# dojo-sim/Dojo.jl

Hardware: NVIDIA H100
Metric: env-steps/sec (forward step!) (higher is better)
Workload: dtype f64

## Files before the change

### dojo.jl_b200/csrc/dojo_b200.cu

```cuda
#include <cuda_runtime.h>

#include <algorithm>
#include <climits>
#include <cstdio>
#include <cstdlib>
#include <cstring>
#include <string>
#include <vector>

#include "../../include/dojo_b200.h"
#include "dojo_step_kernel.cuh"
#include "dojo_kin.cuh"
#include "dojo_kinjac.cuh"
#include "dojo_envs.cuh"
#include "dojo_storage.cuh"

using namespace dj;

extern "C" __attribute__((visibility("hidden"))) const void* dojo_cm_step_kernel(int grad);
static const void* step_kernel_fn(bool any_contact, bool grad, bool plan_smem, bool small = false) {
  if (any_contact) return dojo_cm_step_kernel(grad ? 1 : 0);
  if (plan_smem && !getenv("DOJO_B200_GENERIC_PLAN")) {
    if (!grad && small) return (const void*)dojo_step_kernel<false, true, false, true>;
    return grad ? (const void*)dojo_step_kernel<true, true> : (const void*)dojo_step_kernel<false, true>;
// ... 390 lines not shown
    auto slot_entry = [&](const JointDev& J, int slot) { return (J.flags & JF_FULL) ? (slot | (1 << 30)) : slot; };
    ilist.push_back(slot_entry(joints[parent_joint[b]], joints[parent_joint[b]].slot_c));
    for (int j = 0; j < Ne; ++j) if (joints[j].parent == b) ilist.push_back(slot_entry(joints[j], joints[j].slot_p));
    bodies[b].g_cnt = (int)ilist.size() - bodies[b].g_off;
  }

  for (int b = 0; b < Nb; ++b) {
    bodies[b].pjoint = parent_joint[b];
    bodies[b].cj_off = (int)ilist.size();
    for (int j = 0; j < Ne; ++j) if (joints[j].parent == b) ilist.push_back(j);
    bodies[b].cj_cnt = (int)ilist.size() - bodies[b].cj_off;
    bodies[b].ct_off = (int)ilist.size();
    for (int c = 0; c < Ni; ++c) if (contacts[c].body == b) ilist.push_back(c);
    bodies[b].ct_cnt = (int)ilist.size() - bodies[b].ct_off;
  }

  std::vector<WarpRole> roles(nw);
  {
    for (auto& r : roles) std::memset(&r, 0, sizeof(r));
    auto add = [&](int w, int type, int first, int count) {
      if (count <= 0) return;
      WarpRole& r = roles[w];
      r.type[r.npass] = type; r.first[r.npass] = first; r.count[r.npass] = count; r.npass++;
    };
    if (nw == 1) { add(0, ROLE_BODY, 0, Nb); add(0, ROLE_CONTACT, 0, Ni); add(0, ROLE_JOINT, 0, Ne); }
    else if (nw == 2) { add(0, ROLE_BODY, 0, Nb); add(0, ROLE_CONTACT, 0, Ni); add(1, ROLE_JOINT, 0, Ne); }
    else if (nw == 4) {
      const int hb = (Nb + 1) / 2, hc = (Ni + 1) / 2, hj = (Ne + 1) / 2;
      add(0, ROLE_BODY, 0, hb); add(0, ROLE_CONTACT, 0, hc);
      add(1, ROLE_BODY, hb, Nb - hb); add(1, ROLE_CONTACT, hc, Ni - hc);
      add(2, ROLE_JOINT, 0, hj); add(3, ROLE_JOINT, hj, Ne - hj);
    }
    else {
      int hb = (Nb + 1) / 2, hc = (Ni + 1) / 2, qj = (Ne + 3) / 4;
      add(0, ROLE_BODY, 0, hb); add(1, ROLE_BODY, hb, Nb - hb);
      add(2, ROLE_CONTACT, 0, hc); add(3, ROLE_CONTACT, hc, Ni - hc);
      for (int q = 0; q < 4; ++q) add(4 + q, ROLE_JOINT, q * qj, std::max(0, std::min(qj, Ne - q * qj)));
    }
  }

  struct HStep { ElimStep s; int height; int group; double cost; };
  std::vector<HStep> hs;
  std::vector<int> body_height(Nb, 0);
  {
    std::vector<char> done(Nb, 0);
    struct Rec {
      std::vector<JointDev>& joints; std::vector<BodyDev>& bodies; std::vector<ContactDev>& contacts;
      const std::vector<int>& pj; std::vector<char>& done; std::vector<HStep>& hs; std::vector<int>& ilist; int Ne, Ni;
      int visit(int b) {
        done[b] = 1;
        int hb = 0;
        std::vector<int> fold, gfold;
        for (int j = 0; j < Ne; ++j)
          if (joints[j].parent == b && !done[joints[j].child]) {
            int hc = visit(joints[j].child);
            hb = std::max(hb, hc + 1);
            fold.push_back(joints[j].S_off);
            gfold.push_back(joints[j].gv_off);
          }
        const BodyDev& B = bodies[b];
        const JointDev& J = joints[pj[b]];
        {
          HStep h; std::memset(&h, 0, sizeof(h));
          ElimStep& s = h.s;
          s.d_off = B.D_off; s.n = 6; s.vec_off = B.sol_off; s.r_off = B.r_off; s.nnb = 0;
          s.fold_off = (int)ilist.size(); s.fold_cnt = (int)fold.size();
          for (int f : fold) ilist.push_back(f);
          s.gfold_off = (int)ilist.size();
          for (int f : gfold) ilist.push_back(f);
          int ij = -1, ip = -1;
          if (joint_nq(J) > 0) {
            ij = s.nnb++;
            s.nb[ij].n = joint_nq(J); s.nb[ij].vec_off = J.sol_off; s.nb[ij].r_off = J.r_off; s.nb[ij].gv_off = -1; s.nb[ij].fwd_abs = -1; s.nb[ij].L_off = J.Uc_off; s.nb[ij].U_off = J.Lc_off; s.nb[ij].U_k = 6; s.nb[ij].U_row = 0;
            s.nb[ij].ld = joint_nq(J); s.nb[ij].row0 = 0;
          }
          int r0 = 0;
          if (J.parent >= 0 && J.BBpc_off >= 0) {
            ip = s.nnb++;
            const BodyDev& Pb = bodies[J.parent];
            r0 = (J.flags & JF_FULL) ? 0 : 3;
            s.nb[ip].n = 6 - r0; s.nb[ip].vec_off = Pb.sol_off + r0; s.nb[ip].r_off = Pb.r_off + r0; s.nb[ip].gv_off = J.gv_off; s.nb[ip].fwd_abs = J.S_off + 36 + r0;
            s.nb[ip].L_off = J.BBpc_off; s.nb[ip].U_off = J.BBcp_off; s.nb[ip].U_k = 6 - r0; s.nb[ip].U_row = r0;
            s.nb[ip].ld = 6; s.nb[ip].row0 = r0;
          }
          if (ij >= 0) s.tgt[ij][ij] = J.D_off;
          if (ip >= 0) s.tgt[ip][ip] = J.S_off + 7 * r0;
          if (ij >= 0 && ip >= 0) { s.tgt[ij][ip] = J.Up_off + r0; s.tgt[ip][ij] = J.Lp_off + r0 * joint_nq(J); }
          h.height = hb; h.group = -1; h.cost = 4.0 + joint_nq(J) * 0.3;
          hs.push_back(h);
        }
        int hj = hb;
        if (joint_nq(J) > 0) {
          HStep h; std::memset(&h, 0, sizeof(h));
          ElimStep& s = h.s;
          s.d_off = J.D_off; s.n = joint_nq(J); s.vec_off = J.sol_off; s.r_off = J.r_off; s.nnb = 0;
          if (J.parent >= 0) {
            const BodyDev& Pb = bodies[J.parent];
            s.nnb = 1;
            s.nb[0].n = 6; s.nb[0].vec_off = Pb.sol_off; s.nb[0].r_off = Pb.r_off; s.nb[0].gv_off = J.gv_off; s.nb[0].fwd_abs = J.S_off + 36; s.nb[0].L_off = J.Lp_off; s.nb[0].U_off = J.Up_off; s.nb[0].U_k = joint_nq(J); s.nb[0].U_row = 0;
            s.nb[0].ld = 6; s.nb[0].row0 = 0;
            s.tgt[0][0] = J.S_off;
          }
          hj = hb + 1;
          h.height = hj; h.group = -1; h.cost = 2.0 + joint_nq(J) * 0.4;
          hs.push_back(h);
        }
        return hj;
      }
    } rec{joints, bodies, contacts, parent_joint, done, hs, ilist, Ne, Ni};
    for (int j = 0; j < Ne; ++j) if (joints[j].parent < 0 && !done[joints[j].child]) rec.visit(joints[j].child);
    for (int b = 0; b < Nb; ++b) if (!done[b]) { delete h; return fail("mechanism is not a tree rooted at the origin"); }
  }
  int nphase = 0;
  for (auto& x : hs) nphase = std::max(nphase, x.height + 1);
  std::vector<ElimStep> steps;
  std::vector<int> sched((size_t)nphase * nw * 2, 0);
  for (int ph = 0; ph < nphase; ++ph) {
    std::vector<std::vector<int>> per_warp(nw);
    std::vector<double> load(nw, 0.0);
    std::vector<int> group_warp(Nb, -1);
    for (int i = 0; i < (int)hs.size(); ++i) {
      if (hs[i].height != ph) continue;
      int w;
      if (hs[i].group >= 0 && group_warp[hs[i].group] >= 0) w = group_warp[hs[i].group];
      else {
        w = 0;
        for (int k = 1; k < nw; ++k) if (load[k] < load[w]) w = k;
        if (hs[i].group >= 0) group_warp[hs[i].group] = w;
      }
      per_warp[w].push_back(i);
      load[w] += hs[i].cost;
    }
    for (int w = 0; w < nw; ++w) {
      sched[2 * (ph * nw + w)] = (int)steps.size();
      sched[2 * (ph * nw + w) + 1] = (int)per_warp[w].size();
      for (int i : per_warp[w]) steps.push_back(hs[i].s);
    }
  }
  P.nphase = nphase;
  h->nsteps = (int)steps.size();
  {
    std::vector<int> cnt((size_t)nphase * nw), wfirst(nw);
    std::vector<LduOp> ops;
    bool fits = true;
    auto u16 = [&](int v) { fits = fits && v >= 0 && v < kLduNone; return v & 0xffff; };
    auto u8 = [&](int v) { fits = fits && v >= 0 && v < 256; return v & 0xff; };
    for (int w = 0; w < nw; ++w) {
      wfirst[w] = (int)ops.size();
      for (int ph = 0; ph < nphase; ++ph) {
        const int s0 = sched[2 * (ph * nw + w)], sn = sched[2 * (ph * nw + w) + 1];
        cnt[ph * nw + w] = sn;
        for (int s = s0; s < s0 + sn; ++s) {
          const ElimStep& st = steps[s];
          int f[kLduFold] = {0, 0, 0};
          for (int k = 0; k < std::min(st.fold_cnt, kLduFold); ++k) f[k] = ilist[st.fold_off + k];
          LduOp op;
          std::memset(&op, 0, sizeof(op));
          op.w[0] = u16(st.d_off) | u16(st.vec_off) << 16;
          op.w[1] = u8(st.n) | u8(st.nnb) << 8 | u16(st.fold_cnt) << 16;
          op.w[2] = u16(st.fold_off) | u16(f[0]) << 16;
          op.w[3] = u16(f[1]) | u16(f[2]) << 16;
          for (int i = 0; i < st.nnb; ++i) {
            const ElimNb& nb = st.nb[i];
            int* q = op.w + 4 * (1 + i);
            q[0] = u16(nb.L_off) | (nb.fwd_abs >= 0 ? u16(nb.fwd_abs) : kLduNone) << 16;
            q[1] = u16(nb.vec_off) | u16(nb.U_off) << 16;
            q[2] = u8(nb.n) | u8(nb.U_row) << 8 | u8(nb.U_k) << 16 | u8(nb.ld) << 24;
            q[3] = u16(st.tgt[i][0]) | (st.nnb > 1 ? u16(st.tgt[i][1]) : 0) << 16;
          }
          ops.push_back(op);
        }
      }
    }
    if (!fits) { delete h; return fail("the block LDU program does not fit its 16-bit offsets"); }
    P.prog_cnt = (int)sched.size();
    sched.insert(sched.end(), cnt.begin(), cnt.end());
    sched.insert(sched.end(), wfirst.begin(), wfirst.end());
    sched.resize((sched.size() + 3) & ~size_t(3), 0);
    P.prog_ops = (int)sched.size();
    const int* words = reinterpret_cast<const int*>(ops.data());
    sched.insert(sched.end(), words, words + ops.size() * (sizeof(LduOp) / sizeof(int)));
  }

  cudaDeviceProp prop;
  if (cudaGetDeviceProperties(&prop, device) != cudaSuccess) { delete h; g_create_error = "cudaGetDeviceProperties failed"; return DOJO_ECUDA; }
  h->sm_count = prop.multiProcessorCount;
  if (h->arena_bytes > (size_t)prop.sharedMemPerBlockOptin) {
    delete h;
    g_create_error = "dojo_create: mechanism does not fit the per-environment shared-memory arena";
    return DOJO_ENOMEM;
  }
  auto upload = [&](const void* src, size_t bytes, void** dst) -> bool {
    if (bytes == 0) { *dst = nullptr; return true; }
    if (cudaMalloc(dst, bytes) != cudaSuccess) return false;
    return cudaMemcpy(*dst, src, bytes, cudaMemcpyHostToDevice) == cudaSuccess;
  };
  std::vector<char> blob;
  {
    const void* src[8] = {bodies.data(), joints.data(), contacts.data(), steps.data(), sched.data(), ilist.data(), roles.data(), ucol.data()};
    const size_t len[8] = {sizeof(BodyDev) * Nb, sizeof(JointDev) * Ne, sizeof(ContactDev) * Ni, sizeof(ElimStep) * steps.size(), sizeof(int) * sched.size(),
                           sizeof(int) * ilist.size(), sizeof(WarpRole) * roles.size(), sizeof(int) * ucol.size()};
    const int order[8] = {4, 3, 5, 6, 7, 0, 2, 1};
    for (int q = 0; q < 8; ++q) {
      const int k = order[q];
      h->blob_off[k] = (int)blob.size();
      blob.insert(blob.end(), (const char*)src[k], (const char*)src[k] + len[k]);
      blob.resize((blob.size() + 15) & ~size_t(15), 0);
      h->blob_end[k] = (int)blob.size();
    }
    h->blob_bytes = (int)blob.size();
  }
  bool ok = upload(blob.data(), blob.size(), (void**)&h->d_blob);
  {
    std::vector<int> order;
    std::vector<char> placed(Nb, 0), used(Ne, 0);
    for (bool progress = true; progress && (int)order.size() < Ne;) {
      progress = false;
      for (int j = 0; j < Ne; ++j)
        if (!used[j] && (joints[j].parent < 0 || placed[joints[j].parent])) { order.push_back(j); used[j] = 1; placed[joints[j].child] = 1; progress = true; }
    }
    ok = ok && (int)order.size() == Ne && upload(order.data(), sizeof(int) * Ne, (void**)&h->d_kin_order);
  }
  ok = ok && cudaMalloc((void**)&h->d_counter, sizeof(int)) == cudaSuccess;
  ok = ok && cudaMalloc((void**)&h->d_order, sizeof(int) * max_batch) == cudaSuccess && cudaMalloc((void**)&h->d_prev_iters, sizeof(int32_t) * max_batch) == cudaSuccess &&
       cudaMemset(h->d_prev_iters, 0, sizeof(int32_t) * max_batch) == cudaSuccess;
  if (const char* e = getenv("DOJO_B200_LPT")) { h->lpt = atoi(e) != 0; h->lpt_mode = atoi(e); }
  ok = ok && cudaMalloc((void**)&h->d_key, sizeof(int32_t) * max_batch) == cudaSuccess;
  ok = ok && cudaMalloc((void**)&h->d_prof, (32 + 2 * (size_t)max_batch) * sizeof(unsigned long long)) == cudaSuccess && cudaMemset(h->d_prof, 0, 32 * sizeof(unsigned long long)) == cudaSuccess &&
       cudaMemset(h->d_prof + 31, 0xff, sizeof(unsigned long long)) == cudaSuccess;
  ok = ok && cudaStreamCreateWithFlags(&h->stream, cudaStreamNonBlocking) == cudaSuccess;
  ok = ok && cudaEventCreateWithFlags(&h->ev_last, cudaEventDisableTiming) == cudaSuccess;
  auto pick_slots = [&](size_t bytes) {
    int g = (int)std::min<size_t>((size_t)prop.sharedMemPerBlockOptin / bytes, (size_t)(256 / (32 * nw)));
    g = std::max(1, std::min(g, 8));
    if (const char* e = getenv("DOJO_B200_SLOTS")) { int v = atoi(e); if (v >= 1 && v <= g) g = v; }
    return g;
  };
  h->slots = pick_slots(h->arena_bytes);
  const bool smem_plan = !getenv("DOJO_B200_GLOBAL_PLAN");
  auto plan_prefix = [&](int n, size_t bytes, int* off, int* pbytes, int* mask) {
    *off = -1; *pbytes = 0; *mask = 0;
    if (!smem_plan) return;
    const size_t room = (size_t)prop.sharedMemPerBlockOptin - 1024 - n * bytes;
    for (int k = 0; k < 8; ++k)
      if ((size_t)h->blob_end[k] <= room) { *mask |= 1 << k; *pbytes = std::max(*pbytes, h->blob_end[k]); }
    for (int k = 0; k < 8; ++k)
      if (((*mask >> k) & 1) && h->blob_end[k] > *pbytes) *mask &= ~(1 << k);
    if (*mask) *off = (int)(n * bytes / sizeof(double));
  };
  plan_prefix(h->slots, h->arena_bytes, &h->plan_smem_off, &h->plan_smem_bytes, &h->plan_smem_mask);
  h->smem_fwd = h->slots * h->arena_bytes + h->plan_smem_bytes;
  h->small_step = small_step_ok(h, h->plan_smem_mask);
  h->k_fwd = step_kernel_fn(h->any_contact, false, h->plan_smem_mask == 0xff, h->small_step);
  h->k_grad = step_kernel_fn(h->any_contact, true, false);
  ok = ok && max_shared_memory(h->k_fwd, device) == cudaSuccess;
  const bool grad_fits = h->grad_bytes <= (size_t)prop.sharedMemPerBlockOptin;
  if (grad_fits) {
    h->slots_grad = pick_slots(h->grad_bytes);
    plan_prefix(h->slots_grad, h->grad_bytes, &h->plan_smem_off_grad, &h->plan_smem_bytes_grad, &h->plan_smem_mask_grad);
    h->smem_grad = h->slots_grad * h->grad_bytes + h->plan_smem_bytes_grad;
    h->k_grad = step_kernel_fn(h->any_contact, true, h->plan_smem_mask_grad == 0xff);
    ok = ok && max_shared_memory(h->k_grad, device) == cudaSuccess;
  } else h->grad_bytes = 0;
  if (!ok) { g_create_error = std::string("dojo_create: device allocation failed: ") + cudaGetErrorString(cudaGetLastError()); dojo_destroy(h); return DOJO_ECUDA; }
  P.bodies = (const BodyDev*)(h->d_blob + h->blob_off[0]); P.joints = (const JointDev*)(h->d_blob + h->blob_off[1]);
  P.contacts = (const ContactDev*)(h->d_blob + h->blob_off[2]); P.steps = (const ElimStep*)(h->d_blob + h->blob_off[3]);
  P.sched = (const int*)(h->d_blob + h->blob_off[4]); P.ilist = (const int*)(h->d_blob + h->blob_off[5]);
  P.roles = (const WarpRole*)(h->d_blob + h->blob_off[6]); P.ucol = (const int*)(h->d_blob + h->blob_off[7]);
  int occ = 1;
  cudaOccupancyMaxActiveBlocksPerMultiprocessor(&occ, h->k_fwd, 32 * h->nw * h->slots, h->smem_fwd);
  h->envs_per_sm = std::max(1, occ);
  if (h->grad_bytes) { occ = 1; cudaOccupancyMaxActiveBlocksPerMultiprocessor(&occ, h->k_grad, 32 * h->nw * h->slots_grad, h->smem_grad); h->envs_per_sm_grad = std::max(1, occ); }
  *out = h;
  return DOJO_OK;
}

extern "C" int dojo_destroy(DojoHandle* h) {
  if (!h) return DOJO_OK;
  cudaSetDevice(h->device);
  cudaFree(h->d_key); cudaFree(h->d_order); cudaFree(h->d_prev_iters); cudaFree(h->d_prof); cudaFree(h->d_blob); cudaFree(h->d_counter); cudaFree(h->d_kin_order); cudaFree(h->d_kjws); cudaFree(h->d_kjout); cudaFree(h->d_recZ[0]); cudaFree(h->d_recZ[1]); cudaFree(h->d_recS); cudaFree(h->d_recD); cudaFree(h->d_recAny); cudaFree(h->d_envTheta); cudaFree(h->d_envNorm); cudaFree(h->d_envS); cudaFree(h->d_envSn); cudaFree(h->d_envA); cudaFree(h->d_envR); cudaFree(h->d_envS0); cudaFree(h->d_envDone); cudaFree(h->d_X); cudaFree(h->d_Xn); cudaFree(h->d_gsol); cudaFree(h->d_gstatus); cudaFree(h->d_done); cudaFree(h->d_trace);
  for (int k = 0; k < 2; ++k) { cudaFree(h->d_Fz[k]); cudaFree(h->d_Fu[k]); if (h->ev_kernel[k]) cudaEventDestroy(h->ev_kernel[k]); if (h->ev_copy[k]) cudaEventDestroy(h->ev_copy[k]); }
  if (h->copy_stream) cudaStreamDestroy(h->copy_stream);
  cudaFree(h->d_Z); cudaFree(h->d_U); cudaFree(h->d_F); cudaFree(h->d_Zn); cudaFree(h->d_sol); cudaFree(h->d_status); cudaFree(h->d_iters);
  if (h->p_in) cudaFreeHost(h->p_in);
  if (h->p_out) cudaFreeHost(h->p_out);
  if (h->stream) cudaStreamDestroy(h->stream);
  if (h->ev_last) cudaEventDestroy(h->ev_last);
  cudaFree(h->d_rollU); cudaFree(h->d_rollTraj);
  cudaFree(h->d_rsol); cudaFree(h->d_rdone); cudaFree(h->d_rstatus); cudaFree(h->d_riters); cudaFree(h->d_rZ); cudaFree(h->d_rU); cudaFree(h->d_rX);
  delete h;
  return DOJO_OK;
}

extern "C" const char* dojo_last_error(const DojoHandle* h) { return h ? h->err.c_str() : g_create_error.c_str(); }
extern "C" int dojo_num_state(const DojoHandle* h) { return h->plan.nz; }
extern "C" int dojo_num_input(const DojoHandle* h) { return h->plan.nu; }
extern "C" int dojo_num_residual(const DojoHandle* h) { return h->plan.nres; }
extern "C" int dojo_num_grad_state(const DojoHandle* h) { return 12 * h->plan.Nb; }
extern "C" int dojo_shared_bytes_per_env(const DojoHandle* h) { return (int)h->arena_bytes; }
extern "C" int64_t dojo_launch_count(const DojoHandle* h) { return h->launches; }
extern "C" int dojo_debug_config(const DojoHandle* h, int* out) {
  if (!h || !out) return DOJO_EINVAL;
  const int v[17] = {h->slots, h->slots_grad, h->plan.ch, (int)h->arena_bytes, (int)h->grad_bytes, (int)h->smem_fwd, (int)h->smem_grad,
                     h->plan_smem_mask, h->plan_smem_mask_grad, h->plan.ls_pair, h->plan.nphase, h->nsteps, h->blob_bytes, h->nw, h->envs_per_sm,
                     h->envs_per_sm_grad, h->small_step ? 1 : 0};
  for (int i = 0; i < 17; ++i) out[i] = v[i];
// ... 1224 lines not shown
```

### dojo.jl_b200/csrc/dojo_kernels.cuh

```cuda
#pragma once
#include "dojo_linalg.cuh"
#include "dojo_plan.h"

namespace dj {

#ifdef DJ_ANY_CONTACT
#define DJ_SLOT_OFF(raw) ((raw) & 0x3fffffff)
#define DJ_SLOT_FULL(raw) (((raw) >> 30) & 1)
#else
#define DJ_SLOT_OFF(raw) (raw)
#endif
#ifdef DJ_ANY_CONTACT
DJ_DEV int contact_type(const ContactDev& cd) { return cd.tn & 0xff; }
DJ_DEV int contact_nh(const ContactDev& cd) { return cd.tn >> 8; }
#endif

DJ_DEV V3 ld3(const double* p) { return V3{p[0], p[1], p[2]}; }
DJ_DEV void st3(double* p, V3 v) { p[0] = v.x; p[1] = v.y; p[2] = v.z; }
DJ_DEV void add3(double* p, V3 v) { p[0] += v.x; p[1] += v.y; p[2] += v.z; }
DJ_DEV M33 ldm33(const double* p) {
  M33 r;
#pragma unroll
  for (int i = 0; i < 3; ++i)
#pragma unroll
// ... 1009 lines not shown
      const LimitSide ls = limit_side(so[is_u], so[is_l], so[ig_u], so[ig_l]);
      const double* lim = A + jd.lim_off + kLim * i;
      const double adw = dot(ld3(lim), wp) + dot(ld3(lim + 3), wc);
      const double dgA = xr[is_u], rcI = xr[is_l], rs_u = xr[ig_u], rs_l = xr[ig_l];
      const double ds_u = rs_u - adw, ds_l = rs_l + adw;
      const double dgI = (rcI - ls.gI * (ls.up ? ds_l : ds_u)) / ls.sI;
      xr[is_u] = ds_u;
      xr[is_l] = ds_l;
      xr[ig_u] = ls.up ? dgA : dgI;
      xr[ig_l] = ls.up ? dgI : dgA;
    }
  }
}

template <bool JAC, bool SMALL = false>
DJ_DEV void evaluate(Ctx& c, double f, int res_off, double& rvio, double& bvio) {
  const Plan& P = *c.P;
  double* A = c.A;
  double* res = A + res_off;
  const WarpRole& role = c.roles[c.warp];
  double rv = 0.0, bv = 0.0;
  if (JAC) {
    for (int t = c.tid; t < P.mat_len; t += c.nthreads) A[P.mat_off + t] = 0.0;
    slot_sync(c);
  }
  for (int p = 0; p < role.npass; ++p) {
    if (JAC && role.type[p] == ROLE_JOINT && (SMALL || (P.jpair && role.count[p] <= 16))) {
      if ((c.lane >> 1) < role.count[p]) eval_joint_pair(c, role.first[p] + (c.lane >> 1), (c.lane & 1) != 0, res, rv, bv);
      continue;
    }
    const int idx = role_item(role, p, c.lane);
    if (idx < 0) continue;
    if (role.type[p] == ROLE_BODY) eval_body<JAC>(c, idx, f, res);
    else if (role.type[p] == ROLE_CONTACT) eval_contact<JAC>(c, idx, f, res, rv, bv);
    else if (!(SMALL && JAC)) eval_joint<JAC>(c, idx, f, res, rv, bv);
  }
#ifdef DJ_PROFILE
  long long _rw0 = clock64();
#endif
  slot_sync(c);
#ifdef DJ_PROFILE
  c.t_rolewait += clock64() - _rw0;
#endif
  for (int p = 0; p < role.npass; ++p) {
    const int idx = role_item(role, p, c.lane);
    if (idx < 0 || role.type[p] != ROLE_BODY) continue;
    const BodyDev& bd = c.bodies[idx];
    double* rb = res + bd.sol_off;
    double* D = A + bd.D_off;
    for (int g = 0; g < bd.g_cnt; ++g) {
      const double* s = A + DJ_SLOT_OFF(c.ilist[bd.g_off + g]);
      add3(rb, ld3(s));
      add3(rb + 3, ld3(s + 3));
      if (JAC) {
#ifdef DJ_ANY_CONTACT
        if (g < bd.g_ncontact || DJ_SLOT_FULL(c.ilist[bd.g_off + g])) {
#else
        if (g < bd.g_ncontact) {
#endif
#pragma unroll
          for (int i = 0; i < 36; ++i) D[i] -= s[6 + i];
        } else {
#pragma unroll
          for (int i = 0; i < 3; ++i)
#pragma unroll
            for (int j = 0; j < 3; ++j) D[(3 + i) * 6 + 3 + j] -= s[6 + 3 * i + j];
        }
      }
    }
#pragma unroll
    for (int i = 0; i < 6; ++i) rv = nanmax(rv, fabs(rb[i]));
  }
  block_nanmax2<SMALL>(c, rv, bv);
  rvio = rv;
  bvio = bv;
  slot_sync(c);
}

template <bool SMALL = false>
DJ_DEV void evaluate_ls(Ctx& c, double* W, double fk, bool pair, double& rvA, double& bvA, double& rvB, double& bvB) {
  const Plan& P = *c.P;
  double* A = c.A;
  const WarpRole& role = c.roles[c.warp];
  const bool pl = SMALL || P.ls_pair != 0;
  const int half = pl ? (c.lane >> 4) : 0;
  const int ln = pl ? (c.lane & 15) : c.lane;
  const bool on = (half == 0) || pair;
  const double f = half ? 0.5 * fk : fk;
  double* res = W + (half ? P.ls_res2_off : P.sav_off);
  c.sd = (int)(W - A) + (half ? P.ls_slot_delta : 0);
  double rv = 0.0, bv = 0.0;
  for (int p = 0; p < role.npass; ++p) {
    const int idx = on ? role_item(role, p, ln) : -1;
    if (idx < 0) continue;
    if (role.type[p] == ROLE_BODY) eval_body<false>(c, idx, f, res);
    else if (role.type[p] == ROLE_CONTACT) eval_contact<false>(c, idx, f, res, rv, bv);
    else eval_joint<false>(c, idx, f, res, rv, bv);
  }
  slot_sync(c);
  for (int p = 0; p < role.npass; ++p) {
    const int idx = on ? role_item(role, p, ln) : -1;
    if (idx < 0 || role.type[p] != ROLE_BODY) continue;
    const BodyDev& bd = c.bodies[idx];
    double* rb = res + bd.sol_off;
    for (int g = 0; g < bd.g_cnt; ++g) {
      const double* s = A + DJ_SLOT_OFF(c.ilist[bd.g_off + g]) + c.sd;
      add3(rb, ld3(s));
      add3(rb + 3, ld3(s + 3));
    }
#pragma unroll
    for (int i = 0; i < 6; ++i) rv = nanmax(rv, fabs(rb[i]));
  }
  c.sd = 0;
#pragma unroll
  for (int o = 8; o > 0; o >>= 1) {
    rv = nanmax(rv, __shfl_xor_sync(0xffffffffu, rv, o));
    bv = nanmax(bv, __shfl_xor_sync(0xffffffffu, bv, o));
  }
  if (!pl) {
    rv = nanmax(rv, __shfl_xor_sync(0xffffffffu, rv, 16));
    bv = nanmax(bv, __shfl_xor_sync(0xffffffffu, bv, 16));
  }
  double* red = W + P.red_off;
  if ((c.lane & 15) == 0) { red[4 * c.warp + 2 * (c.lane >> 4)] = rv; red[4 * c.warp + 2 * (c.lane >> 4) + 1] = bv; }
  slot_sync(c);
  rvA = red[0]; bvA = red[1]; rvB = red[2]; bvB = red[3];
  for (int w = 1; w < slot_warps<SMALL>(c); ++w) {
    rvA = nanmax(rvA, red[4 * w]); bvA = nanmax(bvA, red[4 * w + 1]);
    rvB = nanmax(rvB, red[4 * w + 2]); bvB = nanmax(bvB, red[4 * w + 3]);
  }
  slot_sync(c);
}

DJ_DEV const int* ldu_cnt(const Ctx& c) { return c.sched + c.P->prog_cnt; }
DJ_DEV const int4* ldu_op(const Ctx& c, int k) { return reinterpret_cast<const int4*>(c.sched + c.P->prog_ops) + 3 * k; }
DJ_DEV int ldu_fold(const Ctx& c, int4 h, int j) {
  return j == 0 ? hi16(h.z) : j == 1 ? lo16(h.w) : j == 2 ? hi16(h.w) : c.ilist[lo16(h.z) + j];
}
static_assert(kLduFold == 3, "ldu_fold names three inline fold sources");

template <bool SMALL = false>
DJ_DEV bool factorize(Ctx& c) {
  const Plan& P = *c.P;
  double* A = c.A;
  bool ok = true;
  const int half = c.lane >> 4, l = c.lane & 15;
  const unsigned mask = 0xffffu << (16 * half);
  const int nw = slot_warps<SMALL>(c);
  const int* cnt = ldu_cnt(c);
  int k = cnt[P.nphase * nw + c.warp];
#ifdef DJ_PROFILE
  c.f_last = clock64();
#endif
  for (int ph = 0; ph < P.nphase; ++ph) {
    const int sn = cnt[ph * nw + c.warp];
    for (int s = half; s < sn; s += 2) {
      const int4* q = ldu_op(c, k + s);
      const int4 h = q[0];
      const int n = byte_of(h.y, 0), nnb = byte_of(h.y, 1), fold_cnt = hi16(h.y);
      double* Dc = A + lo16(h.x);
      if (fold_cnt > 0) {
        for (int t = l; t < n * n; t += 16) {
          double acc = Dc[t];
          for (int j = 0; j < fold_cnt; ++j) acc += A[ldu_fold(c, h, j) + t];
          Dc[t] = acc;
        }
        __syncwarp(mask);
      }
      DJ_FTICK(c, f_fold)
      ok = block_inverse(Dc, n, n, l, mask) && ok;
      DJ_FTICK(c, f_inv)
      for (int i = 0; i < nnb; ++i) {
        const int4 a = q[1 + i];
        right_multiply_inplace(A + lo16(a.x), Dc, byte_of(a.z, 0), n, l, mask);
      }
      DJ_FTICK(c, f_rm)
      for (int i = 0; i < nnb; ++i)
        for (int j = 0; j < nnb; ++j) {
          const int4 ai = q[1 + i], aj = q[1 + j];
          schur_update(A + (j ? hi16(ai.w) : lo16(ai.w)), byte_of(aj.z, 3), A + lo16(ai.x) + byte_of(aj.z, 1), n, A + hi16(aj.y), byte_of(ai.z, 0),
                       byte_of(aj.z, 2), byte_of(aj.z, 0), l, mask);
        }
      DJ_FTICK(c, f_schur)
    }
    k += sn;
    slot_sync(c);
    DJ_FTICK(c, f_bar)
  }
  int* flag = (int*)(A + P.red_off);
  const bool wok = __all_sync(0xffffffffu, ok);
  if (c.lane == 0) flag[c.warp] = wok ? 1 : 0;
  slot_sync(c);
  bool all = true;
  for (int w = 0; w < slot_warps<SMALL>(c); ++w) all = all && (flag[w] != 0);
  slot_sync(c);
  return all;
}

DJ_DEV double dot6(const double* a, const double* b, int n) {
  double e = 0.0, o = 0.0;
#pragma unroll
  for (int k = 0; k < 6; k += 2) {
    if (k < n) e = fma(a[k], b[k], e);
    if (k + 1 < n) o = fma(a[k + 1], b[k + 1], o);
  }
  return e + o;
}

template <bool SMALL = false>
DJ_DEV void solve(Ctx& c, int vec_off) {
  const Plan& P = *c.P;
  double* A = c.A;
  double* x = A + vec_off;
  const int lane = c.lane;
  const int half = lane >> 4, l = lane & 15;
  const int sub = l >> 3, li = l & 7;
  const WarpRole& role = c.roles[c.warp];
#ifdef DJ_PROFILE
  c.f_last = clock64();
#endif
  for (int p = 0; p < role.npass; ++p) {
    const int idx = role_item(role, p, lane);
    if (idx < 0) continue;
    if (role.type[p] == ROLE_CONTACT) condense_contact(c, idx, x);
    else if (role.type[p] == ROLE_JOINT) condense_joint(c, idx, x);
  }
  DJ_FTICK(c, s_cond)
  slot_sync(c);
  DJ_FTICK(c, s_bar)
  for (int p = 0; p < role.npass; ++p) {
    const int idx = role_item(role, p, lane);
    if (idx < 0 || role.type[p] != ROLE_BODY) continue;
    const BodyDev& bd = c.bodies[idx];
    double* xb = x + bd.sol_off;
    for (int g = 0; g < bd.g_cnt; ++g) {
      const double* s = A + DJ_SLOT_OFF(c.ilist[bd.g_off + g]);
      add3(xb, ld3(s));
      add3(xb + 3, ld3(s + 3));
    }
  }
  DJ_FTICK(c, s_cond)
  slot_sync(c);
  DJ_FTICK(c, s_bar)
  const int nw = slot_warps<SMALL>(c);
  const int* cnt = ldu_cnt(c);
  int k = cnt[P.nphase * nw + c.warp];
  for (int ph = 0; ph < P.nphase; ++ph) {
    const int sn = cnt[ph * nw + c.warp];
    for (int it = 0; 2 * it < sn; ++it) {
      const bool act = 2 * it + half < sn;
      const int4* q = ldu_op(c, k + 2 * it + (act ? half : 0));
      const int4 h = q[0];
      const int n = byte_of(h.y, 0), fold_cnt = hi16(h.y);
      double* xc = x + hi16(h.x);
      if (act && fold_cnt > 0 && l < n) {
        double acc = xc[l];
        for (int j = 0; j < fold_cnt; ++j) {
          double* v = A + ldu_fold(c, h, j) + 36;
          acc += v[l];
          v[l] = 0.0;
        }
        xc[l] = acc;
      }
      __syncwarp();
      if (act && sub < byte_of(h.y, 1)) {
        const int4 a = q[1 + sub];
        if (li < byte_of(a.z, 0)) {
          const double* L = A + lo16(a.x) + li * n;
          const double acc = dot6(L, xc, n);
          double* tgt = hi16(a.x) != kLduNone ? A + hi16(a.x) : x + lo16(a.y);
          tgt[li] -= acc;
        }
      }
      __syncwarp();
    }
    k += sn;
    DJ_FTICK(c, s_fwd)
    slot_sync(c);
    DJ_FTICK(c, s_bar)
  }
  for (int ph = P.nphase - 1; ph >= 0; --ph) {
    const int sn = cnt[ph * nw + c.warp];
    k -= sn;
    for (int it = (sn + 1) / 2 - 1; it >= 0; --it) {
      const bool act = 2 * it + half < sn;
      const int4* q = ldu_op(c, k + 2 * it + (act ? half : 0));
      const int4 h = q[0];
      const int n = byte_of(h.y, 0), nnb = byte_of(h.y, 1);
      const double* Dc = A + lo16(h.x);
      double* xc = x + hi16(h.x);
      if (act && nnb > 0 && l < n) {
        double acc = 0.0;
        for (int j = 0; j < nnb; ++j) {
          const int4 a = q[1 + j];
          const int nn = byte_of(a.z, 0), r = l - byte_of(a.z, 1);
          if (r >= 0 && r < byte_of(a.z, 2)) {
            acc += dot6(A + hi16(a.y) + r * nn, x + lo16(a.y), nn);
          }
        }
        xc[l] -= acc;
      }
      __syncwarp();
      double acc = 0.0;
      if (act && l < n) acc = dot6(Dc + l * n, xc, n);
      __syncwarp();
      if (act && l < n) xc[l] = acc;
      __syncwarp();
    }
    DJ_FTICK(c, s_bwd)
    slot_sync(c);
    DJ_FTICK(c, s_bar)
  }
  for (int p = 0; p < role.npass; ++p) {
    const int idx = role_item(role, p, lane);
    if (idx < 0) continue;
    if (role.type[p] == ROLE_CONTACT) recover_contact(c, idx, x);
    else if (role.type[p] == ROLE_JOINT) recover_joint(c, idx, x);
  }
  DJ_FTICK(c, s_rec)
  slot_sync(c);
  DJ_FTICK(c, s_bar)
}

DJ_DEV double ort_step(double lam, double dl, double tau) { return dl < 0.0 ? fmin(1.0, -tau * lam / dl) : 1.0; }
DJ_DEV double soc_step(double l0, double l1, double l2, double d0, double d1, double d2, double tau) {
  const double eps = 1e-14;
  double ll = fmax(l0 * l0 - (l1 * l1 + l2 * l2), 1e-25) + eps;
  double ld = l0 * d0 - (l1 * d1 + l2 * d2) + eps;
  double rs = ld / ll;
  double sq = sqrt(ll);
  double fct = (ld / sq + d0) / (l0 / sq + 1.0);
  double r1 = d1 / sq - fct * l1 / ll;
  double r2 = d2 / sq - fct * l2 / ll;
  double nr = sqrt(r1 * r1 + r2 * r2);
  return (nr - rs > 0.0) ? fmin(1.0, tau / (nr - rs)) : 1.0;
}
template <bool SMALL = false>
DJ_DEV double cone_line_search(Ctx& c, double tau_ort, double tau_soc) {
  const Plan& P = *c.P;
  const double* sol = c.A + P.sol_off;
  const double* dl = c.A + P.rhs_off;
  const WarpRole& role = c.roles[c.warp];
  double a = 1.0;
  for (int p = 0; p < role.npass; ++p) {
#ifndef DJ_ANY_CONTACT
    if (role.type[p] == ROLE_CONTACT && role.count[p] <= 16) {
      const int ci = c.lane >> 1;
      if (ci < role.count[p]) {
        const ContactDev& cd = c.contacts[role.first[p] + ci];
        const int o = cd.sol_off + 4 * (c.lane & 1);
        const double* v = sol + o;
        const double* dv = dl + o;
        a = fmin(a, ort_step(v[0], dv[0], tau_ort));
        a = fmin(a, soc_step(v[1], v[2], v[3], dv[1], dv[2], dv[3], tau_soc));
      }
      continue;
    }
#endif
    const int idx = role_item(role, p, c.lane);
    if (idx < 0) continue;
    if (role.type[p] == ROLE_CONTACT) {
      const ContactDev& cd = c.contacts[idx];
      const double* s = sol + cd.sol_off;
#ifdef DJ_ANY_CONTACT
      if (contact_type(cd) != 2) {
        const int n2 = 2 * contact_nh(cd);
        for (int i = 0; i < n2; ++i) a = fmin(a, ort_step(s[i], dl[cd.sol_off + i], tau_ort));
        continue;
      }
#endif
      const double* g = s + 4;
      const double* ds = dl + cd.sol_off;
      const double* dg = ds + 4;
      a = fmin(a, ort_step(s[0], ds[0], tau_ort));
      a = fmin(a, ort_step(g[0], dg[0], tau_ort));
      a = fmin(a, soc_step(s[1], s[2], s[3], ds[1], ds[2], ds[3], tau_soc));
      a = fmin(a, soc_step(g[1], g[2], g[3], dg[1], dg[2], dg[3], tau_soc));
    } else if (role.type[p] == ROLE_JOINT) {
      const JointDev& jd = c.joints[idx];
      for (int i = 0; i < 2 * jd.nb_r; ++i) a = fmin(a, ort_step(sol[jd.sol_off + jd.ne + i], dl[jd.sol_off + jd.ne + i], tau_ort));
    }
  }
  return block_min<SMALL>(c, a);
}

template <bool SMALL = false>
DJ_DEV void centering(Ctx& c, double aaff, double& nu, double& nuaff) {
  const Plan& P = *c.P;
  const double* sol = c.A + P.sol_off;
  const double* dl = c.A + P.rhs_off;
  const WarpRole& role = c.roles[c.warp];
  double sn = 0.0, sa = 0.0, cnt = 0.0;
  for (int p = 0; p < role.npass; ++p) {
    const int idx = role_item(role, p, c.lane);
    if (idx < 0) continue;
    if (role.type[p] == ROLE_CONTACT) {
      const ContactDev& cd = c.contacts[idx];
#ifdef DJ_ANY_CONTACT
      if (contact_type(cd) != 2) {
        const int nh = contact_nh(cd);
        for (int i = 0; i < nh; ++i) {
          double s = sol[cd.sol_off + i], g = sol[cd.sol_off + nh + i];
          sn += s * g;
          sa += (s + aaff * dl[cd.sol_off + i]) * (g + aaff * dl[cd.sol_off + nh + i]);
        }
        cnt += (double)nh;
        continue;
      }
#endif
#pragma unroll
      for (int i = 0; i < 4; ++i) {
        double s = sol[cd.sol_off + i], g = sol[cd.sol_off + 4 + i];
        sn += s * g;
        sa += (s + aaff * dl[cd.sol_off + i]) * (g + aaff * dl[cd.sol_off + 4 + i]);
      }
      cnt += 2.0;
    } else if (role.type[p] == ROLE_JOINT) {
      const JointDev& jd = c.joints[idx];
      for (int i = 0; i < jd.nb_r; ++i) {
        int is = jd.sol_off + jd.ne + i, ig = is + jd.nb_r;
        sn += sol[is] * sol[ig];
        sa += (sol[is] + aaff * dl[is]) * (sol[ig] + aaff * dl[ig]);
      }
      cnt += (double)jd.nb_r;
    }
  }
  block_sum3<SMALL>(c, sn, sa, cnt);
  nu = sn / cnt;
  nuaff = sa / cnt;
}

DJ_DEV void correction(Ctx& c) {
  const Plan& P = *c.P;
  const double* dl = c.A + P.rhs_off;
  double* sav = c.A + P.sav_off;
  const WarpRole& role = c.roles[c.warp];
  for (int p = 0; p < role.npass; ++p) {
    const int idx = role_item(role, p, c.lane);
    if (idx < 0) continue;
    if (role.type[p] == ROLE_CONTACT) {
      const ContactDev& cd = c.contacts[idx];
      const double* ds = dl + cd.sol_off;
#ifdef DJ_ANY_CONTACT
      if (contact_type(cd) != 2) {
        const int nh = contact_nh(cd);
        for (int i = 0; i < nh; ++i) sav[cd.sol_off + i] += -ds[i] * ds[nh + i] + c.mu;
        continue;
      }
#endif
      const double* dg = ds + 4;
      double* r = sav + cd.sol_off;
      r[0] += -ds[0] * dg[0] + c.mu;
      r[1] += -(ds[1] * dg[1] + ds[2] * dg[2] + ds[3] * dg[3]) + c.mu;
      r[2] += -(ds[1] * dg[2] + dg[1] * ds[2]);
      r[3] += -(ds[1] * dg[3] + dg[1] * ds[3]);
    } else if (role.type[p] == ROLE_JOINT) {
      const JointDev& jd = c.joints[idx];
      for (int i = 0; i < jd.nb_r; ++i) {
        int is = jd.sol_off + jd.ne + i;
        sav[is] += -dl[is] * dl[is + jd.nb_r] + c.mu;
      }
// ... 173 lines not shown
```

### dojo.jl_b200/csrc/dojo_linalg.cuh

```cuda
#pragma once
#include "dojo_math.cuh"

#ifndef DJ_NOINLINE_LA
#define DJ_LA __device__ __forceinline__
#else
#define DJ_LA __device__ __noinline__
#endif

namespace dj {

template <int N>
DJ_LA bool block_inverse_nopivot_t(double* A, int ld, int l, unsigned mask) {
  static_assert(2 * N <= 16, "block too large for the one-column-per-lane inverse");
  double a[N];
  const bool left = l < N;
  const int col = left ? l : l - N;
  const bool active = l < 2 * N;
#pragma unroll
  for (int r = 0; r < N; ++r) a[r] = active ? (left ? A[r * ld + col] : (r == col ? 1.0 : 0.0)) : 0.0;
  bool ok = true;
#pragma unroll
  for (int k = 0; k < N; ++k) {
#ifdef DJ_BLOCK_PIVOT
    if (k + 1 < N) {
      int p = k;
      double best = fabs(a[k]);
#pragma unroll
      for (int r = k + 1; r < N; ++r) {
        const double v = fabs(a[r]);
        if (v > best) { best = v; p = r; }
      }
      p = __shfl_sync(mask, p, k, 16);
#pragma unroll
      for (int r = k + 1; r < N; ++r)
        if (r == p) { const double t = a[k]; a[k] = a[r]; a[r] = t; }
    }
#endif
    double piv = __shfl_sync(mask, a[k], k, 16);
    if (!(fabs(piv) > 1e-300) || !(fabs(piv) < 1e300)) ok = false;
    double akk = a[k] * (1.0 / piv);
#pragma unroll
    for (int r = 0; r < N; ++r) {
      if (r == k) continue;
      double f = __shfl_sync(mask, a[r], k, 16);
      a[r] -= f * akk;
    }
    a[k] = akk;
  }
  __syncwarp(mask);
  if (active && !left) {
#pragma unroll
    for (int r = 0; r < N; ++r) A[r * ld + col] = a[r];
  }
  __syncwarp(mask);
  return ok;
}

DJ_DEV bool block_inverse(double* A, int n, int ld, int l, unsigned mask) {
  switch (n) {
    case 1: return block_inverse_nopivot_t<1>(A, ld, l, mask);
    case 2: return block_inverse_nopivot_t<2>(A, ld, l, mask);
    case 3: return block_inverse_nopivot_t<3>(A, ld, l, mask);
    case 4: return block_inverse_nopivot_t<4>(A, ld, l, mask);
    case 5: return block_inverse_nopivot_t<5>(A, ld, l, mask);
    case 6: return block_inverse_nopivot_t<6>(A, ld, l, mask);
    default: return false;
  }
}

__device__ __noinline__ void right_multiply_generic(double* L, const double* Dinv, int m, int n, int l, unsigned mask) {
  const int total = m * n;
  double out[3];
#pragma unroll
  for (int p = 0; p < 3; ++p) {
    int e = l + 16 * p;
    double acc = 0.0;
    if (e < total) {
      int i = e / n, j = e - i * n;
      for (int k = 0; k < n; ++k) acc += L[i * n + k] * Dinv[k * n + j];
    }
    out[p] = acc;
  }
  __syncwarp(mask);
#pragma unroll
  for (int p = 0; p < 3; ++p) {
    int e = l + 16 * p;
    if (e < total) L[e] = out[p];
  }
  __syncwarp(mask);
}

__device__ __noinline__ void schur_generic(double* C, int ldc, const double* A, int lda, const double* B, int ni, int k, int nj, int l, unsigned mask) {
  const int total = ni * nj;
  for (int e = l; e < total; e += 16) {
    int i = e / nj, j = e - i * nj;
    double acc = 0.0;
    for (int t = 0; t < k; ++t) acc += A[i * lda + t] * B[t * nj + j];
    C[i * ldc + j] -= acc;
  }
  __syncwarp(mask);
}

constexpr int kStrip = 3;

template <int M, int N>
DJ_LA void right_multiply_t(double* L, const double* Dinv, int l, unsigned mask) {
  constexpr int SPR = (N + kStrip - 1) / kStrip;
  constexpr int NS = M * SPR;
  static_assert(NS <= 16, "single pass only");
  const int i = l / SPR, js = (l - i * SPR) * kStrip;
  double acc[kStrip] = {0.0, 0.0, 0.0};
  if (l < NS) {
#pragma unroll
    for (int k = 0; k < N; ++k) {
      double a = L[i * N + k];
#pragma unroll
      for (int c = 0; c < kStrip; ++c)
        if (js + c < N) acc[c] += a * Dinv[k * N + js + c];
    }
  }
  __syncwarp(mask);
  if (l < NS) {
#pragma unroll
    for (int c = 0; c < kStrip; ++c)
      if (js + c < N) L[i * N + js + c] = acc[c];
  }
  __syncwarp(mask);
}

template <int NI, int K, int NJ, int LDC = NJ>
DJ_LA void schur_t(double* C, const double* A, int lda, const double* B, int l, unsigned mask) {
  constexpr int SPR = (NJ + kStrip - 1) / kStrip;
  constexpr int NS = NI * SPR;
  static_assert(NS <= 16, "single pass only");
  if (l < NS) {
    const int i = l / SPR, js = (l - i * SPR) * kStrip;
    double acc[kStrip] = {0.0, 0.0, 0.0};
#pragma unroll
    for (int t = 0; t < K; ++t) {
      double a = A[i * lda + t];
#pragma unroll
      for (int c = 0; c < kStrip; ++c)
        if (js + c < NJ) acc[c] += a * B[t * NJ + js + c];
    }
#pragma unroll
    for (int c = 0; c < kStrip; ++c)
      if (js + c < NJ) C[i * LDC + js + c] -= acc[c];
  }
  __syncwarp(mask);
}

#define DJ_RM_CASE(M, N) case (M) * 32 + (N): right_multiply_t<M, N>(L, Dinv, l, mask); return;
DJ_DEV void right_multiply_inplace(double* L, const double* Dinv, int m, int n, int l, unsigned mask) {
  switch (m * 32 + n) {
    DJ_RM_CASE(6, 6) DJ_RM_CASE(5, 6) DJ_RM_CASE(6, 5) DJ_RM_CASE(3, 6) DJ_RM_CASE(6, 3)
    default: right_multiply_generic(L, Dinv, m, n, l, mask);
  }
}
#define DJ_SC_CASE(NI, K, NJ) case (((NI) * 32 + (K)) * 32 + (NJ)) * 8 + (NJ): schur_t<NI, K, NJ>(C, A, lda, B, l, mask); return;
#define DJ_SC_CASE_LD6(NI, K, NJ) case (((NI) * 32 + (K)) * 32 + (NJ)) * 8 + 6: schur_t<NI, K, NJ, 6>(C, A, lda, B, l, mask); return;
DJ_DEV void schur_update(double* C, int ldc, const double* A, int lda, const double* B, int ni, int k, int nj, int l, unsigned mask) {
  switch (((ni * 32 + k) * 32 + nj) * 8 + ldc) {
    DJ_SC_CASE(6, 6, 6)
    DJ_SC_CASE(5, 6, 5) DJ_SC_CASE(5, 6, 6) DJ_SC_CASE(6, 6, 5) DJ_SC_CASE(6, 5, 6)
    DJ_SC_CASE(3, 6, 3) DJ_SC_CASE(3, 6, 6) DJ_SC_CASE(6, 6, 3) DJ_SC_CASE(6, 3, 6)
    DJ_SC_CASE_LD6(6, 3, 3) DJ_SC_CASE_LD6(5, 3, 3) DJ_SC_CASE_LD6(3, 3, 3) DJ_SC_CASE(3, 6, 5)
    default: schur_generic(C, ldc, A, lda, B, ni, k, nj, l, mask);
  }
}

}
```

Before: 482,900.

## Fuse fold into block inverse and make triangular solves register/shuffle based

The factorization now folds the contributions of neighbouring blocks directly into the registers used by the block inverse, instead of doing a separate pass through shared memory followed by a sync. It also prefetches each phase's first op header. The forward and backward solves preload L, D and U rows into registers and broadcast the pivot vector with half-warp shuffles. This removes several __syncwarp calls and shared-memory round trips per elimination step. The host plan is also restricted to at most two neighbours per step, since the backward solve now hard-codes two neighbour slots; this adds register pressure and speculative loads.

```diff
diff --git a/dojo.jl_b200/csrc/dojo_b200.cu b/dojo.jl_b200/csrc/dojo_b200.cu
--- a/dojo.jl_b200/csrc/dojo_b200.cu
+++ b/dojo.jl_b200/csrc/dojo_b200.cu
@@ -566,6 +566,7 @@
         cnt[ph * nw + w] = sn;
         for (int s = s0; s < s0 + sn; ++s) {
           const ElimStep& st = steps[s];
+          fits = fits && st.nnb <= 2;
           int f[kLduFold] = {0, 0, 0};
           for (int k = 0; k < std::min(st.fold_cnt, kLduFold); ++k) f[k] = ilist[st.fold_off + k];
           LduOp op;
diff --git a/dojo.jl_b200/csrc/dojo_kernels.cuh b/dojo.jl_b200/csrc/dojo_kernels.cuh
--- a/dojo.jl_b200/csrc/dojo_kernels.cuh
+++ b/dojo.jl_b200/csrc/dojo_kernels.cuh
@@ -1185,23 +1185,16 @@
 #ifdef DJ_PROFILE
   c.f_last = clock64();
 #endif
+  int sn = cnt[c.warp];
+  int4 h0 = half < sn ? ldu_op(c, k + half)[0] : int4{};
   for (int ph = 0; ph < P.nphase; ++ph) {
-    const int sn = cnt[ph * nw + c.warp];
     for (int s = half; s < sn; s += 2) {
       const int4* q = ldu_op(c, k + s);
-      const int4 h = q[0];
+      const int4 h = s == half ? h0 : q[0];
       const int n = byte_of(h.y, 0), nnb = byte_of(h.y, 1), fold_cnt = hi16(h.y);
       double* Dc = A + lo16(h.x);
-      if (fold_cnt > 0) {
-        for (int t = l; t < n * n; t += 16) {
-          double acc = Dc[t];
-          for (int j = 0; j < fold_cnt; ++j) acc += A[ldu_fold(c, h, j) + t];
-          Dc[t] = acc;
-        }
-        __syncwarp(mask);
-      }
       DJ_FTICK(c, f_fold)
-      ok = block_inverse(Dc, n, n, l, mask) && ok;
+      ok = block_inverse(Dc, n, n, l, mask, fold_cnt, [&](int j) { return A + ldu_fold(c, h, j); }) && ok;
       DJ_FTICK(c, f_inv)
       for (int i = 0; i < nnb; ++i) {
         const int4 a = q[1 + i];
@@ -1217,6 +1210,10 @@
       DJ_FTICK(c, f_schur)
     }
     k += sn;
+    if (ph + 1 < P.nphase) {
+      sn = cnt[(ph + 1) * nw + c.warp];
+      if (half < sn) h0 = ldu_op(c, k + half)[0];
+    }
     slot_sync(c);
     DJ_FTICK(c, f_bar)
   }
@@ -1230,7 +1227,8 @@
   return all;
 }
 
-DJ_DEV double dot6(const double* a, const double* b, int n) {
+template <class VA, class VB>
+DJ_DEV double dot6(const VA& a, const VB& b, int n) {
   double e = 0.0, o = 0.0;
 #pragma unroll
   for (int k = 0; k < 6; k += 2) {
@@ -1238,6 +1236,11 @@
     if (k + 1 < n) o = fma(a[k + 1], b[k + 1], o);
   }
   return e + o;
+}
+
+DJ_DEV void group6(double z, double (&v)[6]) {
+#pragma unroll
+  for (int t = 0; t < 6; ++t) v[t] = __shfl_sync(0xffffffffu, z, t, 16);
 }
 
 template <bool SMALL = false>
@@ -1278,68 +1281,78 @@
   const int nw = slot_warps<SMALL>(c);
   const int* cnt = ldu_cnt(c);
   int k = cnt[P.nphase * nw + c.warp];
+  int sn = cnt[c.warp];
   for (int ph = 0; ph < P.nphase; ++ph) {
-    const int sn = cnt[ph * nw + c.warp];
     for (int it = 0; 2 * it < sn; ++it) {
       const bool act = 2 * it + half < sn;
       const int4* q = ldu_op(c, k + 2 * it + (act ? half : 0));
       const int4 h = q[0];
+      const int4 a = q[1 + sub];
       const int n = byte_of(h.y, 0), fold_cnt = hi16(h.y);
+      const bool prod = act && sub < byte_of(h.y, 1) && li < byte_of(a.z, 0);
+      double Lr[6];
+      const double* L = A + lo16(a.x) + li * n;
+#pragma unroll
+      for (int j = 0; j < 6; ++j) Lr[j] = prod && j < n ? L[j] : 0.0;
       double* xc = x + hi16(h.x);
-      if (act && fold_cnt > 0 && l < n) {
-        double acc = xc[l];
+      double z = 0.0;
+      if (act && l < n) {
+        z = xc[l];
         for (int j = 0; j < fold_cnt; ++j) {
           double* v = A + ldu_fold(c, h, j) + 36;
-          acc += v[l];
+          z += v[l];
           v[l] = 0.0;
         }
-        xc[l] = acc;
-      }
-      __syncwarp();
-      if (act && sub < byte_of(h.y, 1)) {
-        const int4 a = q[1 + sub];
-        if (li < byte_of(a.z, 0)) {
-          const double* L = A + lo16(a.x) + li * n;
-          const double acc = dot6(L, xc, n);
-          double* tgt = hi16(a.x) != kLduNone ? A + hi16(a.x) : x + lo16(a.y);
-          tgt[li] -= acc;
-        }
-      }
-      __syncwarp();
+        if (fold_cnt > 0) xc[l] = z;
+      }
+      double zc[6];
+      group6(z, zc);
+      if (prod) {
+        const double acc = dot6(Lr, zc, n);
+        double* tgt = hi16(a.x) != kLduNone ? A + hi16(a.x) : x + lo16(a.y);
+        tgt[li] -= acc;
+      }
     }
     k += sn;
+    if (ph + 1 < P.nphase) sn = cnt[(ph + 1) * nw + c.warp];
     DJ_FTICK(c, s_fwd)
     slot_sync(c);
     DJ_FTICK(c, s_bar)
   }
   for (int ph = P.nphase - 1; ph >= 0; --ph) {
-    const int sn = cnt[ph * nw + c.warp];
     k -= sn;
     for (int it = (sn + 1) / 2 - 1; it >= 0; --it) {
       const bool act = 2 * it + half < sn;
       const int4* q = ldu_op(c, k + 2 * it + (act ? half : 0));
-      const int4 h = q[0];
+      const int4 h = q[0], a0 = q[1], a1 = q[2];
       const int n = byte_of(h.y, 0), nnb = byte_of(h.y, 1);
-      const double* Dc = A + lo16(h.x);
+      const bool row = act && l < n;
+      double Dr[6], M0[6], x0[6], M1[6], x1[6];
+      const double* Dc = A + lo16(h.x) + l * n;
+#pragma unroll
+      for (int t = 0; t < 6; ++t) Dr[t] = row && t < n ? Dc[t] : 0.0;
       double* xc = x + hi16(h.x);
-      if (act && nnb > 0 && l < n) {
-        double acc = 0.0;
-        for (int j = 0; j < nnb; ++j) {
-          const int4 a = q[1 + j];
-          const int nn = byte_of(a.z, 0), r = l - byte_of(a.z, 1);
-          if (r >= 0 && r < byte_of(a.z, 2)) {
-            acc += dot6(A + hi16(a.y) + r * nn, x + lo16(a.y), nn);
-          }
-        }
-        xc[l] -= acc;
-      }
-      __syncwarp();
+      const double zl = row ? xc[l] : 0.0;
+      const int nn0 = byte_of(a0.z, 0), r0 = l - byte_of(a0.z, 1), nn1 = byte_of(a1.z, 0), r1 = l - byte_of(a1.z, 1);
+      const bool u0 = row && nnb > 0 && r0 >= 0 && r0 < byte_of(a0.z, 2);
+      const bool u1 = row && nnb > 1 && r1 >= 0 && r1 < byte_of(a1.z, 2);
+#pragma unroll
+      for (int t = 0; t < 6; ++t) {
+        M0[t] = u0 && t < nn0 ? A[hi16(a0.y) + r0 * nn0 + t] : 0.0;
+        x0[t] = u0 && t < nn0 ? x[lo16(a0.y) + t] : 0.0;
+        M1[t] = u1 && t < nn1 ? A[hi16(a1.y) + r1 * nn1 + t] : 0.0;
+        x1[t] = u1 && t < nn1 ? x[lo16(a1.y) + t] : 0.0;
+      }
       double acc = 0.0;
-      if (act && l < n) acc = dot6(Dc + l * n, xc, n);
-      __syncwarp();
-      if (act && l < n) xc[l] = acc;
-      __syncwarp();
-    }
+      if (u0) acc += dot6(M0, x0, nn0);
+      if (u1) acc += dot6(M1, x1, nn1);
+      const double z = nnb > 0 ? zl - acc : zl;
+      double zc[6];
+      group6(z, zc);
+      const double xl = dot6(Dr, zc, n);
+      if (row) xc[l] = xl;
+    }
+    if (ph > 0) sn = cnt[(ph - 1) * nw + c.warp];
     DJ_FTICK(c, s_bwd)
     slot_sync(c);
     DJ_FTICK(c, s_bar)
diff --git a/dojo.jl_b200/csrc/dojo_linalg.cuh b/dojo.jl_b200/csrc/dojo_linalg.cuh
--- a/dojo.jl_b200/csrc/dojo_linalg.cuh
+++ b/dojo.jl_b200/csrc/dojo_linalg.cuh
@@ -9,8 +9,8 @@
 
 namespace dj {
 
-template <int N>
-DJ_LA bool block_inverse_nopivot_t(double* A, int ld, int l, unsigned mask) {
+template <int N, class Fold>
+DJ_LA bool block_inverse_nopivot_t(double* A, int ld, int l, unsigned mask, int nfold, const Fold& fold) {
   static_assert(2 * N <= 16, "block too large for the one-column-per-lane inverse");
   double a[N];
   const bool left = l < N;
@@ -18,6 +18,12 @@
   const bool active = l < 2 * N;
 #pragma unroll
   for (int r = 0; r < N; ++r) a[r] = active ? (left ? A[r * ld + col] : (r == col ? 1.0 : 0.0)) : 0.0;
+  for (int j = 0; j < nfold; ++j) {
+    const double* F = fold(j);
+#pragma unroll
+    for (int r = 0; r < N; ++r)
+      if (left) a[r] += F[r * ld + col];
+  }
   bool ok = true;
 #pragma unroll
   for (int k = 0; k < N; ++k) {
@@ -56,14 +62,15 @@
   return ok;
 }
 
-DJ_DEV bool block_inverse(double* A, int n, int ld, int l, unsigned mask) {
+template <class Fold>
+DJ_DEV bool block_inverse(double* A, int n, int ld, int l, unsigned mask, int nfold, const Fold& fold) {
   switch (n) {
-    case 1: return block_inverse_nopivot_t<1>(A, ld, l, mask);
-    case 2: return block_inverse_nopivot_t<2>(A, ld, l, mask);
-    case 3: return block_inverse_nopivot_t<3>(A, ld, l, mask);
-    case 4: return block_inverse_nopivot_t<4>(A, ld, l, mask);
-    case 5: return block_inverse_nopivot_t<5>(A, ld, l, mask);
-    case 6: return block_inverse_nopivot_t<6>(A, ld, l, mask);
+    case 1: return block_inverse_nopivot_t<1>(A, ld, l, mask, nfold, fold);
+    case 2: return block_inverse_nopivot_t<2>(A, ld, l, mask, nfold, fold);
+    case 3: return block_inverse_nopivot_t<3>(A, ld, l, mask, nfold, fold);
+    case 4: return block_inverse_nopivot_t<4>(A, ld, l, mask, nfold, fold);
+    case 5: return block_inverse_nopivot_t<5>(A, ld, l, mask, nfold, fold);
+    case 6: return block_inverse_nopivot_t<6>(A, ld, l, mask, nfold, fold);
     default: return false;
   }
 }
```

Measured after the change: 491,800 (median of 6 runs). +1.8%, better.
